# PaddlePaddle/PaddleScience

Hardware: AMD Instinct MI355X
Metric: collocation-points/sec (PDE residual+grad) (higher is better)
Workload: dtype f32

## Files before the change

include/ppsci_hip.h:

```cpp
#ifndef PPSCI_HIP_H
#define PPSCI_HIP_H

#include <stddef.h>
#include <stdint.h>

#ifdef __cplusplus
extern "C" {
#endif

#define PPSCI_MAX_IN 8
#define PPSCI_MAX_DIRS 4
#define PPSCI_MAX_OUT 8
#define PPSCI_MAX_HIDDEN 16
#define PPSCI_MAX_PROG 128
#define PPSCI_MAX_RES 8
#define PPSCI_MAX_EPARAM 8
#define PPSCI_MAX_AUX 16

enum { PPSCI_OK = 0, PPSCI_E_INVALID = -1, PPSCI_E_UNSUPPORTED = -2, PPSCI_E_LAUNCH = -3 };
enum { PPSCI_ACT_TANH = 0, PPSCI_ACT_SILU = 1, PPSCI_ACT_SIN = 2, PPSCI_ACT_SIGMOID = 3, PPSCI_ACT_COS = 4, PPSCI_ACT_GELU = 5,
       PPSCI_ACT_SWISH = 6, PPSCI_ACT_STAN = 7,
       PPSCI_ACT_RELU = 8, PPSCI_ACT_LEAKY_RELU = 9, PPSCI_ACT_ELU = 10, PPSCI_ACT_SELU = 11, PPSCI_ACT_IDENTITY = 12 };
enum { PPSCI_EMBED_NONE = 0, PPSCI_EMBED_PERIOD = 1,
       PPSCI_EMBED_STREAMS = 2 };
// ... 132 lines not shown
int64_t ppsci_taylor_step_workspace_bytes(const ppsci_mlp_desc* d, const ppsci_epilogue_desc* e, int64_t n_points);
int ppsci_taylor_step_kind(const ppsci_mlp_desc* d, const ppsci_epilogue_desc* e, int64_t n_points);
void ppsci_set_fused_step(int on);
void ppsci_set_step_tail(int mode);
void ppsci_set_tail_split(int n);
void ppsci_set_fast_program(int on);
void ppsci_set_static_program(int on);
int ppsci_epilogue_predecode(const ppsci_epilogue_desc* e, uint32_t* out256, int* n_loads);
typedef struct ppsci_step_plan ppsci_step_plan;
ppsci_step_plan* ppsci_taylor_step_plan(const ppsci_mlp_desc* d, const ppsci_epilogue_desc* e, float* params,
                                        int64_t n_points, const float* const* inputs_host, const float* const* aux_host,
                                        float* U, float* Ubar, float* residual_out, void* stash, void* workspace,
                                        int64_t workspace_bytes, float* loss_terms, float* grad);
int ppsci_taylor_step_run(ppsci_step_plan* plan, int accumulate, const ppsci_adam_args* adam, void* stream);
#define PPSCI_STEP_KEEP_FRAGMENTS 1
int ppsci_taylor_step_run_ex(ppsci_step_plan* plan, int accumulate, const ppsci_adam_args* adam, void* stream, int flags);
int ppsci_taylor_step_plan_apply(ppsci_step_plan* plan, const ppsci_adam_args* adam, void* stream);
int ppsci_taylor_step_plan_set_scales(ppsci_step_plan* plan, const ppsci_epilogue_desc* e);
int ppsci_taylor_step_run_main(ppsci_step_plan* plan, void* stream);
void ppsci_taylor_step_plan_free(ppsci_step_plan* plan);
int ppsci_taylor_step_plan_static(const ppsci_step_plan* plan, const char** name);
void ppsci_set_fused_specialised(int on);
int ppsci_taylor_step_plan_specialised(const ppsci_step_plan* plan);
int ppsci_taylor_step(const ppsci_mlp_desc* d, const ppsci_epilogue_desc* e, float* params, int64_t n_points,
                      const float* const* inputs_host, const float* const* aux_host, float* U, float* Ubar,
                      float* residual_out, void* stash, void* workspace, int64_t workspace_bytes, float* loss_terms,
                      float* grad, int accumulate, const ppsci_adam_args* adam, void* stream);

int ppsci_reduce_rows(const float* partials, int64_t rows, int64_t cols, float* out, int accumulate,
                      void* stream);

int ppsci_adam_step(int64_t n, float* params, const float* grad, float* m, float* v, float lr,
                    float beta1, float beta2, float eps, int64_t step_t, float grad_scale,
                    void* stream);

#define PPSCI_MTL_MAX_LOSSES 8
#define PPSCI_MTL_PCGRAD 0
#define PPSCI_MTL_GRAM_ONLY 1
int64_t ppsci_grad_surgery_workspace_bytes(int K, int64_t n);
int ppsci_grad_surgery(int K, int64_t n, const float* G, int64_t ld, const int32_t* order, int mode, float* gram_out,
                       float* coef_out, float* w_out, void* workspace, int64_t workspace_bytes, void* stream);
int ppsci_grad_combine(int K, int64_t n, const float* G, int64_t ld, const float* w_dev, const float* w_host, float* out,
                       float* params, const ppsci_adam_args* adam, void* stream);

#define PPSCI_OPT_SGD 0
#define PPSCI_OPT_MOMENTUM 1
// ... 314 lines not shown
```

paddlescience_amd/_lib.py:

```python
from __future__ import annotations

import ctypes as C
import os
from typing import List, Optional, Sequence

MAX_IN, MAX_DIRS, MAX_OUT, MAX_HIDDEN, MAX_PROG, MAX_RES, MAX_AUX = 8, 4, 8, 16, 128, 8, 16

ACT = {"tanh": 0, "silu": 1, "sin": 2, "sigmoid": 3, "cos": 4, "gelu": 5, "swish": 6, "stan": 7, "relu": 8, "leaky_relu": 9,
       "elu": 10, "selu": 11, "identity": 12}
PARAM_ACTS = ("swish", "stan")
SIREN_W0 = 30.0
LINEAR_PLAIN, LINEAR_WEIGHT_NORM, LINEAR_RWF, LINEAR_FOURIER, LINEAR_BROADCAST = range(5)
LINEAR_PADDED = 100
EMBED_NONE, EMBED_PERIOD, EMBED_STREAMS = 0, 1, 2

(OP_LD_IN, OP_LD_U, OP_LD_AUX, OP_CONST, OP_ADD, OP_SUB, OP_MUL, OP_DIV, OP_NEG, OP_POW, OP_SIN, OP_COS,
 OP_TANH, OP_EXP, OP_LOG, OP_SQRT, OP_ABS, OP_SINH, OP_COSH, OP_TAN, OP_MAX, OP_MIN, OP_SIGN, OP_HEAVISIDE,
 OP_DETACH, OP_ASIN, OP_ACOS, OP_ATAN, OP_ATAN2, OP_ASINH, OP_ACOSH, OP_ATANH, OP_ERF, OP_LGAMMA, OP_CEIL, OP_FLOOR,
 OP_LD_PARAM, OP_COUNT) = range(38)
MAX_EPARAM = 8
MTL_MAX_LOSSES = 8
MTL_PCGRAD, MTL_GRAM_ONLY = 0, 1
STEP_KEEP_FRAGMENTS = 1

# ... 134 lines not shown
                                        C.c_void_p, C.c_void_p]),
    "ppsci_taylor_bwd": (C.c_int, [C.POINTER(MlpDesc), C.c_void_p, C.c_int64, C.POINTER(C.c_void_p), C.c_void_p,
                                   C.c_void_p, C.c_void_p, C.c_void_p, C.c_void_p]),
    "ppsci_taylor_bwd_ws": (C.c_int, [C.POINTER(MlpDesc), C.c_void_p, C.c_int64, C.POINTER(C.c_void_p), C.c_void_p,
                                      C.c_void_p, C.c_void_p, C.c_int64, C.c_void_p, C.c_void_p]),
    "ppsci_dense_matvec": (C.c_int, [C.c_int64, C.c_int64, C.c_void_p, C.c_void_p, C.c_void_p, C.c_float, C.c_int, C.c_void_p,
                                     C.c_void_p]),
    "ppsci_csr_matvec": (C.c_int, [C.c_int64, C.c_int64, C.c_int64, C.c_void_p, C.c_void_p, C.c_void_p, C.c_void_p, C.c_void_p,
                                   C.c_float, C.c_void_p, C.c_void_p]),
    "ppsci_reduce_rows": (C.c_int, [C.c_void_p, C.c_int64, C.c_int64, C.c_void_p, C.c_int, C.c_void_p]),
    "ppsci_taylor_step_workspace_bytes": (C.c_int64, [C.POINTER(MlpDesc), C.POINTER(EpilogueDesc), C.c_int64]),
    "ppsci_taylor_step_kind": (C.c_int, [C.POINTER(MlpDesc), C.POINTER(EpilogueDesc), C.c_int64]),
    "ppsci_set_fused_step": (None, [C.c_int]),
    "ppsci_set_step_tail": (None, [C.c_int]),
    "ppsci_set_tail_split": (None, [C.c_int]),
    "ppsci_set_fast_program": (None, [C.c_int]),
    "ppsci_taylor_step_run_ex": (C.c_int, [C.c_void_p, C.c_int, C.POINTER(AdamArgs), C.c_void_p, C.c_int]),
    "ppsci_taylor_step_plan_apply": (C.c_int, [C.c_void_p, C.POINTER(AdamArgs), C.c_void_p]),
    "ppsci_set_static_program": (None, [C.c_int]),
    "ppsci_epilogue_predecode": (C.c_int, [C.POINTER(EpilogueDesc), C.POINTER(C.c_uint32), C.POINTER(C.c_int)]),
    "ppsci_taylor_step_plan_static": (C.c_int, [C.c_void_p, C.POINTER(C.c_char_p)]),
    "ppsci_set_fused_specialised": (None, [C.c_int]),
    "ppsci_taylor_step_plan_specialised": (C.c_int, [C.c_void_p]),
    "ppsci_taylor_step_plan": (C.c_void_p, [C.POINTER(MlpDesc), C.POINTER(EpilogueDesc), C.c_void_p, C.c_int64,
                                            C.POINTER(C.c_void_p), C.POINTER(C.c_void_p), C.c_void_p, C.c_void_p, C.c_void_p,
                                            C.c_void_p, C.c_void_p, C.c_int64, C.c_void_p, C.c_void_p]),
    "ppsci_taylor_step_run": (C.c_int, [C.c_void_p, C.c_int, C.POINTER(AdamArgs), C.c_void_p]),
    "ppsci_taylor_step_plan_set_scales": (C.c_int, [C.c_void_p, C.POINTER(EpilogueDesc)]),
    "ppsci_taylor_step_run_main": (C.c_int, [C.c_void_p, C.c_void_p]),
    "ppsci_taylor_step_plan_free": (None, [C.c_void_p]),
    "ppsci_taylor_step": (C.c_int, [C.POINTER(MlpDesc), C.POINTER(EpilogueDesc), C.c_void_p, C.c_int64, C.POINTER(C.c_void_p),
                                    C.POINTER(C.c_void_p), C.c_void_p, C.c_void_p, C.c_void_p, C.c_void_p, C.c_void_p,
                                    C.c_int64, C.c_void_p, C.c_void_p, C.c_int, C.POINTER(AdamArgs), C.c_void_p]),
    "ppsci_spectral_conv2d_fwd": (C.c_int, [C.POINTER(SpectralDesc), C.c_void_p, C.c_void_p, C.c_void_p, C.c_void_p,
                                            C.c_void_p]),
    "ppsci_spectral_conv2d_bwd": (C.c_int, [C.POINTER(SpectralDesc), C.c_void_p, C.c_void_p, C.c_void_p, C.c_void_p,
                                            C.c_void_p, C.c_void_p, C.c_void_p, C.c_void_p]),
    "ppsci_spectral_conv2d_bwd_real": (C.c_int, [C.POINTER(SpectralDesc), C.c_void_p, C.c_void_p, C.c_void_p, C.c_void_p,
                                                 C.c_void_p, C.c_void_p, C.c_void_p, C.c_float, C.c_int, C.c_void_p]),
    "ppsci_spectral_conv2d_fwd_scaled": (C.c_int, [C.POINTER(SpectralDesc), C.c_void_p, C.c_void_p, C.c_void_p, C.c_void_p,
                                                   C.c_float, C.c_int, C.c_void_p]),
    "ppsci_spectral_conv2d_bwd_real_scaled": (C.c_int, [C.POINTER(SpectralDesc), C.c_void_p, C.c_void_p, C.c_void_p,
                                                        C.c_void_p, C.c_void_p, C.c_void_p, C.c_void_p, C.c_float, C.c_int,
                                                        C.c_float, C.c_int, C.c_void_p]),
    "ppsci_dft2_kept_supported": (C.c_int, [C.c_int] * 4),
    "ppsci_dft2_kept_fwd": (C.c_int, [C.c_int] * 6 + [C.c_void_p] * 3),
# ... 222 lines not shown
```

paddlescience_amd/csrc/taylor_api.hip:

```cpp
#include "taylor_tile.h"
#include "taylor_step.h"
#include "epi_static.h"

#include <math.h>
#include <stdlib.h>
#include <string.h>

#include <mutex>

__global__ void __launch_bounds__(256) ppsci_presplit_kernel(const float* params, ppsci_derived q, int H, int L, int bwd,
                                                             u32x4* out) {
  const int NB = q.NB, NKP = NB / 2;
  const int per_layer = NB * NKP * 64;
  const int total = (L - 1) * per_layer;
  for (int idx = blockIdx.x * blockDim.x + threadIdx.x; idx < total; idx += gridDim.x * blockDim.x) {
    const int l = 1 + idx / per_layer, rem = idx % per_layer;
    const int lane = rem & 63, pair = rem >> 6, rb = pair / NKP, kp = pair - rb * NKP;
    const int g = lane >> 4, c = lane & 15;
    const float* W = params + q.offW[l];
    ppsci_split4 sp[2];
#pragma unroll
    for (int hlf = 0; hlf < 2; ++hlf) {
      const int kb = 2 * kp + hlf;
      f32x4 v;
// ... 290 lines not shown
  const int64_t other = ppsci_bwd_workspace_bytes(d, n_points);
  int rc;
  if (other > 0 && other <= workspace_bytes) {
    rc = taylor_bwd_impl(d, params, n_points, inputs_host, Ubar, stash, workspace, grad_partials, stream);
  } else {
    ppsci_set_error("taylor_bwd: workspace of %lld bytes, %lld needed (ppsci_bwd_workspace_bytes)", (long long)workspace_bytes,
                    (long long)need);
    rc = PPSCI_E_INVALID;
  }
  ppsci_set_bwd_layerwise(knob);
  return rc;
}

static int g_fused_step = 1, g_step_tail = -1, g_fast_vm = 1, g_static_prog = 1;
extern "C" void ppsci_set_fast_program(int on) { g_fast_vm = on ? 1 : 0; }
extern "C" void ppsci_set_static_program(int on) { g_static_prog = on ? 1 : 0; }
extern "C" int ppsci_epilogue_predecode(const ppsci_epilogue_desc* e, uint32_t* out256, int* n_loads) {
  int nl = 0;
  if (!e || !out256) return -1;
  const int n = epi_fast_encode(*e, out256, &nl);
  if (n_loads) *n_loads = nl;
  return n;
}
static int g_fused_spec = 1;
extern "C" void ppsci_set_fused_specialised(int on) { g_fused_spec = on ? 1 : 0; }
extern "C" void ppsci_set_fused_step(int on) { g_fused_step = on ? 1 : 0; }
extern "C" void ppsci_set_step_tail(int mode) { g_step_tail = (mode < 0 || mode > 3) ? -1 : mode; }
#define PPSCI_FUSED_TREE_MAX_GRID 48

static int run_step_act(StepArgs& a, void* stream, int launch, int* grid) {
  if (a.f.d.fourier_half > 0) return PPSCI_E_UNSUPPORTED;
  if (launch == 2 ? a.t.fused != 0 : g_fused_step != 0) {
    int rc = PPSCI_E_UNSUPPORTED;
    const bool st = a.e.static_id > 0;
    switch (a.f.d.activation) {
      case PPSCI_ACT_TANH: rc = st ? ppsci_fused_static_run_tanh(a, stream, launch, grid) : ppsci_fused_run_tanh(a, stream, launch, grid); break;
      case PPSCI_ACT_SILU: rc = st ? ppsci_fused_static_run_silu(a, stream, launch, grid) : ppsci_fused_run_silu(a, stream, launch, grid); break;
      case PPSCI_ACT_SIN: rc = st ? ppsci_fused_static_run_sin(a, stream, launch, grid) : ppsci_fused_run_sin(a, stream, launch, grid); break;
      default: break;
    }
    if (rc != PPSCI_E_UNSUPPORTED || launch == 2) return rc;
    a.e.static_id = 0;
  }
  a.t.fused = 0;
  switch (a.f.d.activation) {
    case PPSCI_ACT_TANH: return ppsci_step_run_tanh(a, stream, launch, grid);
    case PPSCI_ACT_SILU: return ppsci_step_run_silu(a, stream, launch, grid);
    case PPSCI_ACT_SIN: return ppsci_step_run_sin(a, stream, launch, grid);
// ... 173 lines not shown
    if (nfast >= 0) {
#ifdef PPSCI_EMU
      memcpy(ws + y.fastprog, fast, sizeof(fast));
#else
      if (hipMemcpy(ws + y.fastprog, fast, sizeof(fast), hipMemcpyHostToDevice) != hipSuccess) {
        ppsci_set_error("taylor_step: cannot upload the pre-decoded residual program");
        return fail();
      }
#endif
      a.e.fast = (const unsigned*)(ws + y.fastprog);
      a.e.nfast = nfast;
      a.e.nfast_loads = nfast_loads;
    }
  }
  a.f.params = a.b.params = params;
  for (int j = 0; j < d->d_raw; ++j) a.f.x[j] = a.b.x[j] = a.e.x[j] = inputs_host[j];
  for (int j = 0; j < e->n_aux; ++j) a.e.aux[j] = aux_host[j];
  a.f.U = U;
  a.f.stash = (f32x4*)stash;
  a.e.U = U;
  a.e.Ubar = Ubar;
  a.e.resid = residual_out;
  a.t.spec = (a.t.fused && a.t.spec_ok && g_fused_spec && !U && !Ubar && !residual_out) ? 1 : 0;
  a.e.partials = ws + y.rows_l;
  a.b.Ubar = Ubar;
  a.b.stash = (const f32x4*)stash;
  a.b.partials = ws + y.rows_s;
  a.b.wpart = (f32x4*)(ws + y.rows_w);
  StepTail& t = a.t;
  t.rows_w = ws + y.rows_w;
  t.rows_s = ws + y.rows_s;
  t.rows_l = ws + y.rows_l;
  t.tree = ws + y.tree;
  t.counters = (unsigned*)(ws + y.counters);
  t.grad = grad;
  t.loss_terms = loss_terms;
  t.p = params;
  t.per_tile = y.per_tile;
  t.psmall = y.psmall;
  t.n_res = e->n_res;
  t.rowlen = y.rowlen;
  return plan;
}

extern "C" void ppsci_taylor_step_plan_free(ppsci_step_plan* plan) { delete plan; }

extern "C" int ppsci_taylor_step_plan_static(const ppsci_step_plan* plan, const char** name) {
  const int id = plan ? plan->a.e.static_id : 0;
  if (name) *name = epi_static_name(id);
  return id;
}

extern "C" int ppsci_taylor_step_plan_specialised(const ppsci_step_plan* plan) { return plan && plan->a.t.fused && plan->a.t.spec ? 1 : 0; }

extern "C" int ppsci_taylor_step_plan_set_scales(ppsci_step_plan* plan, const ppsci_epilogue_desc* e) {
  if (!plan || !e || e->n_res != plan->a.e.e.n_res) {
    ppsci_set_error("taylor_step_plan_set_scales: invalid argument");
    return PPSCI_E_INVALID;
  }
  for (int k = 0; k < e->n_res; ++k) plan->a.e.e.res[k].scale = e->res[k].scale;
  return PPSCI_OK;
}

extern "C" int ppsci_taylor_step_run(ppsci_step_plan* plan, int accumulate, const ppsci_adam_args* adam, void* stream) {
  return ppsci_taylor_step_run_ex(plan, accumulate, adam, stream, 0);
}

extern "C" int ppsci_taylor_step_run_ex(ppsci_step_plan* plan, int accumulate, const ppsci_adam_args* adam, void* stream, int flags) {
  if (!plan) {
    ppsci_set_error("taylor_step_run: invalid argument");
    return PPSCI_E_INVALID;
  }
  StepTail& t = plan->a.t;
  t.accumulate = accumulate ? 1 : 0;
  t.do_adam = 0;
  if (adam) {
// ... 141 lines not shown
```

paddlescience_amd/csrc/taylor_fused.inc:

```
#include "taylor_tile.h"
#include "taylor_step_tail.h"
#include "epi_static.h"

#include <stdlib.h>
#include <string.h>
#include <type_traits>

#ifndef PPSCI_FUSED_STATIC
#define PPSCI_FUSED_STATIC 0
#endif
#ifndef PPSCI_FUSED_LANE_BIAS
#define PPSCI_FUSED_LANE_BIAS(L, S, ACT, STATIC) ((L) * ((S) + 1) <= (((STATIC) && (ACT) == PPSCI_ACT_TANH) ? 20 : 12))
#endif
#define PPSCI_FUSED_EPI_SCRATCH ((PPSCI_MAX_RES + PPSCI_MAX_EPARAM) * 16)
#define PPSCI_FUSED_SPEC_TAB (64 + PPSCI_MAX_RES + PPSCI_MAX_DIRS * PPSCI_FUSED_MAX_IN)
#define PPSCI_FUSED_MAX_IN 4
#define PPSCI_FUSED_XJ(x, j) ((j) == 0 ? (x)[0] : ((j) == 1 ? (x)[1] : ((j) == 2 ? (x)[2] : (x)[3])))

#ifdef PPSCI_FUSED_TIMERS
#define PPSCI_FT(k)                                             \
  {                                                             \
    const unsigned long long now_ = __builtin_amdgcn_s_memtime(); \
    tacc[k] += now_ - tlast;                                    \
    tlast = now_;                                               \
  }
#else
#define PPSCI_FT(k)
#endif

#define PPSCI_ABL(n) (((ABL) >> (n)) & 1)
template <int ABL>
__device__ __forceinline__ ppsci_split4 ppsci_fused_split(f32x4 x) {
  if (PPSCI_ABL(6)) {
    ppsci_split4 o;
    o.p[0] = (u32x2){__builtin_bit_cast(unsigned, x[0]), __builtin_bit_cast(unsigned, x[1])};
    o.p[1] = (u32x2){__builtin_bit_cast(unsigned, x[2]), __builtin_bit_cast(unsigned, x[3])};
    o.p[2] = o.p[0];
    return o;
  }
// ... 1 lines not shown
}

#ifdef PPSCI_DBG_DUMP
__device__ float* ppsci_dbg_buf = nullptr;
extern "C" int ppsci_dbg_set(float* p) { return (int)hipMemcpyToSymbol(HIP_SYMBOL(ppsci_dbg_buf), &p, sizeof(p)); }
#define PPSCI_DBG_STRIDE 16384
#endif


static inline long long ppsci_fused_floats(const ppsci_mlp_desc& d, const ppsci_derived& q, int S, int n_instr) {
  const int m = d.d_out, pad4m = ((m + 3) / 4) * 4;
  long long fl = 2LL * ((q.d0 + d.n_hidden + m) * q.HP + pad4m);
  fl += (q.NB + 1) * m * S * PPSCI_TILE;
  fl += q.NB * d.d_raw * PPSCI_TILE;
  fl += (long long)q.NB * m * S * PPSCI_TILE;
  fl += PPSCI_FUSED_EPI_SCRATCH + PPSCI_MAX_RES * PPSCI_TILE;
  fl += 2LL * n_instr * PPSCI_TILE;
  fl += EPI_FAST_WORDS + PPSCI_MAX_RES + PPSCI_MAX_RES * PPSCI_TILE;
  fl += 2LL * S * q.NB * 3 * 64 * 2;
  fl += PPSCI_MAX_DIRS * q.HP;
  return fl;
}

template <int NB, int LH, int N1, int N2, int D_RAW, int M>
static constexpr long long ppsci_fused_floats_spec() {
  constexpr int S = 1 + N1 + N2, HP = 16 * NB, pad4m = ((M + 3) / 4) * 4;
  long long fl = 2LL * ((D_RAW + LH + M) * HP + pad4m);
  fl += 2LL * NB * M * S * PPSCI_TILE;
  fl += NB * D_RAW * PPSCI_TILE;
  fl += PPSCI_FUSED_EPI_SCRATCH + PPSCI_MAX_RES * PPSCI_TILE;
  fl += PPSCI_FUSED_SPEC_TAB;
  fl += 2LL * S * NB * 3 * 64 * 2;
  fl += PPSCI_MAX_DIRS * HP;
  return fl;
}

template <int NB, int LH, int N1, int N2, int ACT, bool STATIC, int ABL = 0, int D_RAW = 0, int M = 0>
__global__ void __launch_bounds__(64 * NB, 2) taylor_fused_kernel(StepArgs args) {
  constexpr int S = 1 + N1 + N2;
  constexpr bool SPEC = D_RAW > 0;
  static_assert(!SPEC || (STATIC && M > 0 && D_RAW <= PPSCI_FUSED_MAX_IN), "shape-specialised kernels are STATIC kernels");
  constexpr int HP = 16 * NB;
  constexpr int W = NB;
  constexpr int L = LH;
  constexpr int NKP = NB / 2;
  constexpr bool LANE_BIAS = PPSCI_FUSED_LANE_BIAS(LH, S, ACT, STATIC);
  static_assert(NB == 4, "one feature block per wave, both k-pairs of a layer's fragments held in registers");
  PPSCI_DYN_SMEM(smem);
  const FwdArgs& a = args.f;
  const int tid = threadIdx.x, nthr = blockDim.x;
  const int lane = tid & 63, wave = __builtin_amdgcn_readfirstlane(tid >> 6);
  const int g = lane >> 4, c = lane & 15;
  const int H = a.d.width, m = SPEC ? M : a.d.d_out, d0 = SPEC ? D_RAW : a.q.d0, d_raw = SPEC ? D_RAW : a.d.d_raw;
  const int pad4m = ((m + 3) / 4) * 4;
  const int n_instr = SPEC ? 0 : args.e.e.n_instr;

  float* W0s = smem;
  float* Bs = W0s + d0 * HP;
  float* WLs = Bs + L * HP;
  float* BLs = WLs + m * HP;
  float* gW0 = BLs + pad4m;
  float* gB = gW0 + d0 * HP;
  float* gWL = gB + L * HP;
  float* gBL = gWL + m * HP;
  float* tin = gBL + pad4m;
  float* uls = tin + W * m * S * PPSCI_TILE;
  float* tinx = uls + (SPEC ? 0 : m * S * PPSCI_TILE);
  float* red = tinx + W * d_raw * PPSCI_TILE;
  float* ered = red + W * m * S * PPSCI_TILE;
  float* lacc = ered + PPSCI_FUSED_EPI_SCRATCH;
  float* rf = lacc + PPSCI_MAX_RES * PPSCI_TILE;
  unsigned* ftab = (unsigned*)(rf + 2 * n_instr * PPSCI_TILE);
  float* rres = (float*)(ftab + EPI_FAST_WORDS + PPSCI_MAX_RES);
  u32x2* zx = (u32x2*)(SPEC ? (float*)ftab + PPSCI_FUSED_SPEC_TAB : rres + PPSCI_MAX_RES * PPSCI_TILE);
  u32x2* hx = zx + S * NB * 3 * 64;
  float* dz0 = (float*)(hx + S * NB * 3 * 64);
  f32x4* zsave = (f32x4*)hx;
  static_assert(L * S * 64 * 16 <= S * NB * 3 * 64 * 8, "zsave must fit into hx");
  constexpr bool VM_REGS_OK = (L - 1) * NB * 64 * 16 <= S * NB * 3 * 64 * 8;
  float* prow = args.b.partials + (long long)blockIdx.x * ppsci_small_params(a.d, a.q);

  for (int idx = tid; idx < d0 * HP; idx += nthr) {
    const int k = idx / HP, f = idx - k * HP;
    W0s[idx] = (f < H) ? a.params[a.q.offW[0] + k * H + f] : 0.f;
  }
  for (int idx = tid; idx < L * HP; idx += nthr) {
    const int l = idx / HP, f = idx - l * HP;
    Bs[idx] = (f < H) ? a.params[a.q.offB[l] + f] : 0.f;
  }
  for (int idx = tid; idx < m * HP; idx += nthr) {
    const int cc = idx / HP, f = idx - cc * HP;
    WLs[idx] = (f < H) ? a.params[a.q.offW[L] + f * m + cc] : 0.f;
  }
  for (int idx = tid; idx < pad4m; idx += nthr) BLs[idx] = idx < m ? a.params[a.q.offB[L] + idx] : 0.f;
  bool raw_only = true;
  if constexpr (!SPEC)
    for (int j = 0; j < d_raw; ++j) raw_only = raw_only && a.d.embed[j] == PPSCI_EMBED_NONE;
  if (raw_only)
    for (int idx = tid; idx < N1 * HP; idx += nthr) {
// ... 116 lines not shown
#pragma unroll
            for (int i = 0; i < N2; ++i) d2v[i] = ddv * a.d.dirs[i][j] * a.d.dirs[i][j];
          }
          const f32x4 w4 = *(const f32x4*)&W0s[k * HP + 16 * wave + 4 * g];
          h[0] += w4 * val;
#pragma unroll
          for (int i = 0; i < N1; ++i) h[1 + i] += w4 * d1v[i];
#pragma unroll
          for (int i = 0; i < N2; ++i) h[1 + N1 + i] += w4 * d2v[i];
        }
      }
      h[0] += *(const f32x4*)&Bs[16 * wave + 4 * g];
    }

    PPSCI_FT(1)
    auto fwd_layer = [&](auto lc) {
      constexpr int l = decltype(lc)::value;
      int lanel = lane;
      PPSCI_OPAQUE(lanel);
      const int g = lanel >> 4;
      const int xcl = ppsci_xchunk(lanel >> 4, lanel & 15);
      if constexpr (l > 0) {
        u32x2* xb = STATIC ? (((L - 1 - l) & 1) ? zx : hx) : ((l & 1) ? zx : hx);
        if constexpr (STATIC && l == 1 && (L % 2) == 0) ppsci_block_sync_lds();
        const u32x4* gf = (const u32x4*)a.xfrag + (long long)(l - 1) * PPSCI_GFRAG_PER_LAYER(NB) + lanel;
        u32x4 Ak[NKP][3];
#pragma unroll
        for (int kp = 0; kp < NKP; ++kp)
#pragma unroll
          for (int q = 0; q < 3; ++q) Ak[kp][q] = gf[((wave * NKP + kp) * 3 + q) * 64];
#pragma unroll
        for (int s = 0; s < S; ++s) {
          const ppsci_split4 sp = ppsci_fused_split<ABL>(h[s]);
#pragma unroll
          for (int q = 0; q < 3; ++q)
            if (!PPSCI_ABL(9) || (sp.p[q][0] == 0x12345u && sp.p[q][1] == 0x54321u)) xb[ppsci_xpair(NB, s, wave, q, xcl)] = sp.p[q];
        }
        __builtin_amdgcn_sched_barrier(0);
        ppsci_block_sync_lds();
        PPSCI_FT(2)
        h[0] = *(const f32x4*)&Bs[l * HP + 16 * wave + 4 * g];
#pragma unroll
        for (int s = 1; s < S; ++s) h[s] = (f32x4){0.f, 0.f, 0.f, 0.f};
        {
          u32x4 bq[2][S];
          const auto load_b = [&](int grp, u32x4 (&dst)[S]) {
            const int kp = grp / 3, pb = 2 - grp % 3;
#pragma unroll
            for (int s = 0; s < S; ++s) dst[s] = *(const u32x4*)&xb[ppsci_xpair(NB, s, 2 * kp, pb, xcl)];
          };
          load_b(0, bq[0]);
#pragma unroll
          for (int grp = 0; grp < 3 * NKP; ++grp) {
            const int kp = grp / 3, pb = 2 - grp % 3;
            if (grp + 1 < 3 * NKP) load_b(grp + 1, bq[(grp + 1) & 1]);
            __builtin_amdgcn_sched_barrier(0);
#pragma unroll
            for (int pa = 2 - pb; pa >= 0; --pa)
#pragma unroll
              for (int s = 0; s < S; ++s) {
                const u32x4 bb = bq[grp & 1][s];
                if (PPSCI_ABL(5)) h[s][0] += __builtin_bit_cast(float, bb[0] ^ Ak[kp][pa][0]) * 1e-30f;
// ... 365 lines not shown
            const int kp = grp / 3, pb = 2 - grp % 3;
            if (grp + 1 < 3 * NKP) load_b(grp + 1, bq[(grp + 1) & 1]);
            __builtin_amdgcn_sched_barrier(0);
#pragma unroll
            for (int pa = 2 - pb; pa >= 0; --pa)
#pragma unroll
              for (int s = 0; s < S; ++s) {
                const u32x4 bb = bq[grp & 1][s];
                if (PPSCI_ABL(4)) hb[s][0] += __builtin_bit_cast(float, bb[0] ^ Ab[kp][pa][0]) * 1e-30f;
                else
                hb[s] = ppsci_xdl32a(Ab[kp][pa], (u32x2){bb[0], bb[1]}, (u32x2){bb[2], bb[3]}, hb[s]);
              }
            __builtin_amdgcn_sched_barrier(0);
          }
        }
#ifdef PPSCI_DBG_DUMP
        if (ppsci_dbg_buf != nullptr && l == L - 1) {
#pragma unroll
          for (int s = 0; s < S; ++s) *(f32x4*)&ppsci_dbg_buf[(long long)blockIdx.x * PPSCI_DBG_STRIDE + 8192 + (s * 256 + tid) * 4] = hb[s];
        }
#endif
        PPSCI_FT(8)
        constexpr bool HPAIR = STATIC && l == L - 1;
        if (!PPSCI_ABL(3) && !HPAIR) {
          f32x4 E1, E2, E3;
          f32x4 hcs[S];
          if (PPSCI_ABL(7)) {
            hcs[0] = zst[l - 1][0];
            E1 = (f32x4){0.5f, 0.5f, 0.5f, 0.5f}, E2 = (f32x4){0.1f, 0.1f, 0.1f, 0.1f};
          } else
            ppsci_act_from_stash4<ACT>(zst[l - 1][0], hcs[0], E1, E2, E3);
#pragma unroll
          for (int i = 0; i < N1; ++i) {
            hcs[1 + i] = E1 * zst[l - 1][1 + i];
            if (i < N2) hcs[1 + N1 + i] = E2 * zst[l - 1][1 + i] * zst[l - 1][1 + i] + E1 * zst[l - 1][1 + N1 + i];
          }
#pragma unroll
          for (int s = 0; s < S; ++s) {
            const ppsci_split4 sp = ppsci_fused_split<ABL>(hcs[s]);
#pragma unroll
            for (int q = 0; q < 3; ++q)
              if (!PPSCI_ABL(9) || (sp.p[q][0] == 0x12345u && sp.p[q][1] == 0x54321u)) hx[((s * NB + wave) * 3 + q) * 64 + xcl] = sp.p[q];
            __builtin_amdgcn_sched_barrier(0);
          }
        }
        __builtin_amdgcn_sched_barrier(0);
        if (!PPSCI_ABL(3)) ppsci_block_sync_lds();
        PPSCI_FT(9)
#pragma unroll 1
        for (int sp = 0; sp + 1 < (PPSCI_ABL(3) ? 0 : S); sp += 2) {
          int zs_ = ppsci_xpair(NB, sp, wave, 0, xtl);
          int hs_ = HPAIR ? ppsci_xpair(NB, sp, 0, 0, xtl) : xtl + sp * NB * 3 * 64;
          PPSCI_OPAQUE(zs_);
          PPSCI_OPAQUE(hs_);
          u32x2 zN0[3], zN1[3];
#pragma unroll
          for (int q = 0; q < 3; ++q) {
            zN0[q] = ppsci_lds_read_tr16(&zx[zs_ + q * 128]);
            zN1[q] = ppsci_lds_read_tr16(&zx[zs_ + (NKP * 3 + q) * 128]);
          }
          constexpr int IG = 2;
          u32x2 hN0[2][IG][3], hN1[2][IG][3];
          const auto load_h = [&](int ig, int buf) {
#pragma unroll
            for (int e = 0; e < IG; ++e)
#pragma unroll
              for (int q = 0; q < 3; ++q) {
                if constexpr (HPAIR) {
                  hN0[buf][e][q] = ppsci_lds_read_tr16(&hx[hs_ + (((ig + e) >> 1) * 3 + q) * 128 + ((ig + e) & 1)]);
                  hN1[buf][e][q] = ppsci_lds_read_tr16(&hx[hs_ + ((NKP + ((ig + e) >> 1)) * 3 + q) * 128 + ((ig + e) & 1)]);
                } else {
                  hN0[buf][e][q] = ppsci_lds_read_tr16(&hx[hs_ + ((ig + e) * 3 + q) * 64]);
                  hN1[buf][e][q] = ppsci_lds_read_tr16(&hx[hs_ + ((NB + ig + e) * 3 + q) * 64]);
                }
              }
          };
          load_h(0, 0);
#pragma unroll
          for (int ig = 0; ig < NB; ig += IG) {
            const int buf = (ig / IG) & 1;
            if (ig + IG < NB) load_h(ig + IG, buf ^ 1);
            __builtin_amdgcn_sched_barrier(0);
#pragma unroll
            for (int q = 0; q < PPSCI_XDL_NPROD; ++q)
#pragma unroll
              for (int e = 0; e < IG; ++e)
                wacc[l - 1][ig + e] = ppsci_xdl32(hN0[buf][e][ppsci_xdl_pa[q]], hN1[buf][e][ppsci_xdl_pa[q]], zN0[ppsci_xdl_pb[q]],
                                                  zN1[ppsci_xdl_pb[q]], wacc[l - 1][ig + e]);
            __builtin_amdgcn_sched_barrier(0);
          }
        }
        if constexpr (S & 1) {
          u32x2 zN0[3];
#pragma unroll
          for (int q = 0; q < 3; ++q) zN0[q] = ppsci_lds_read_tr16(&zx[ppsci_xpair(NB, S - 1, wave, q, xtl)]);
          u32x2 hN0[NB][3];
#pragma unroll
          for (int e = 0; e < NB; ++e)
#pragma unroll
            for (int q = 0; q < 3; ++q)
              hN0[e][q] = ppsci_lds_read_tr16(HPAIR ? &hx[ppsci_xpair(NB, S - 1, e, q, xtl)] : &hx[(((S - 1) * NB + e) * 3 + q) * 64 + xtl]);
#pragma unroll
          for (int q = 0; q < PPSCI_XDL_NPROD; ++q)
#pragma unroll
            for (int e = 0; e < NB; ++e)
              wacc[l - 1][e] = ppsci_xdl16(hN0[e][ppsci_xdl_pa[q]], zN0[ppsci_xdl_pb[q]], wacc[l - 1][e]);
          __builtin_amdgcn_sched_barrier(0);
        }
        PPSCI_FT(10)
      } else {
        PPSCI_FT(7)
        const long long p = (long long)tile * PPSCI_TILE + c;
        const long long pp = p < a.N ? p : 0;
        const float vm = p < a.N ? 1.f : 0.f;
        int k = 0;
        if constexpr (STATIC) {
#pragma unroll
          for (int j = 0; j < PPSCI_FUSED_MAX_IN; ++j) {
            if (j < d_raw && !PPSCI_ABL(0)) {
              f32x4 t = hb[0] * tx[j * PPSCI_TILE + c];
#pragma unroll
              for (int i = 0; i < N1; ++i) t += hb[1 + i] * (SPEC ? dirs_s[i * D_RAW + j] : a.d.dirs[i][j]);
              f32x4 v4;
#pragma unroll
// ... 105 lines not shown
  }
  for (int idx = tid; idx < H * m; idx += nthr) {
    const int f = idx / m, cc = idx - f * m;
    ppsci_store_agent(&prow[(d0 + L) * H + idx], gWL[cc * HP + f]);
  }
  for (int idx = tid; idx < m; idx += nthr) ppsci_store_agent(&prow[(d0 + L + m) * H + idx], gBL[idx]);
  {
    float lsum[PPSCI_MAX_RES], padj[PPSCI_MAX_EPARAM];
#pragma unroll
    for (int k = 0; k < PPSCI_MAX_RES; ++k) lsum[k] = (wave == 0 && lane < PPSCI_TILE) ? lacc[k * PPSCI_TILE + lane] : 0.f;
#pragma unroll
    for (int k = 0; k < PPSCI_MAX_EPARAM; ++k) padj[k] = 0.f;
    epi_finale<EPI_RF_FUSED>(args.e, ered, lsum, padj);
  }
  if (args.t.external != 1) ppsci_step_tail(args.t, args.b.d, args.b.q, smem);
}

#if PPSCI_FUSED_STATIC && defined(PPSCI_FUSED_SPEC_D_RAW) && !defined(PPSCI_ABL_BUILD)
#define PPSCI_FUSED_HAS_SPEC 1
#define PPSCI_FUSED_SPEC_KERNEL (taylor_fused_kernel<NB, LH, N1, N2, PPSCI_ACT_ID, true, 0, PPSCI_FUSED_SPEC_D_RAW, PPSCI_FUSED_SPEC_M>)
#else
#define PPSCI_FUSED_HAS_SPEC 0
#endif

template <int NB, int LH, int N1, int N2>
static int launch_fused(StepArgs& a, void* stream, int launch, int* grid_out) {
  constexpr int S = 1 + N1 + N2;
#if PPSCI_FUSED_HAS_SPEC
  constexpr int lds_spec = (int)(ppsci_fused_floats_spec<NB, LH, N1, N2, PPSCI_FUSED_SPEC_D_RAW, PPSCI_FUSED_SPEC_M>() * 4);
#endif
  if (launch == 2) {
#if PPSCI_FUSED_HAS_SPEC
    if (a.t.spec) {
      PPSCI_LAUNCH(PPSCI_FUSED_SPEC_KERNEL, StepArgs, a.t.grid, 64 * NB, lds_spec, stream, a);
      int e = PPSCI_LAST_LAUNCH_ERROR();
      if (e != 0) {
        ppsci_set_error("taylor_fused: launch failed (hip error %d)", e);
        return PPSCI_E_LAUNCH;
      }
      return PPSCI_OK;
    }
#endif
#ifdef PPSCI_ABL_BUILD
    {
      const char* ev = getenv("PPSCI_ABL");
      const int mask = ev ? atoi(ev) : 0;
#define PPSCI_ABL_CASE(M_)                                                                                                          \
  if (mask == (M_)) {                                                                                                               \
    PPSCI_SET_MAX_LDS((taylor_fused_kernel<NB, LH, N1, N2, PPSCI_ACT_ID, PPSCI_FUSED_STATIC != 0, (M_)>), a.t.lds);                    \
    PPSCI_LAUNCH((taylor_fused_kernel<NB, LH, N1, N2, PPSCI_ACT_ID, PPSCI_FUSED_STATIC != 0, (M_)>), StepArgs, a.t.grid, 64 * NB, a.t.lds, \
                 stream, a);                                                                                                        \
    return PPSCI_LAST_LAUNCH_ERROR() != 0 ? PPSCI_E_LAUNCH : PPSCI_OK;                                                              \
  }
      PPSCI_ABL_CASE(1) PPSCI_ABL_CASE(2) PPSCI_ABL_CASE(4) PPSCI_ABL_CASE(8) PPSCI_ABL_CASE(16) PPSCI_ABL_CASE(32) PPSCI_ABL_CASE(64)
      PPSCI_ABL_CASE(128) PPSCI_ABL_CASE(256) PPSCI_ABL_CASE(512)
#undef PPSCI_ABL_CASE
    }
#endif
    PPSCI_LAUNCH((taylor_fused_kernel<NB, LH, N1, N2, PPSCI_ACT_ID, PPSCI_FUSED_STATIC != 0>), StepArgs, a.t.grid, 64 * NB, a.t.lds, stream, a);
    int e = PPSCI_LAST_LAUNCH_ERROR();
    if (e != 0) {
      ppsci_set_error("taylor_fused: launch failed (hip error %d)", e);
      return PPSCI_E_LAUNCH;
    }
    return PPSCI_OK;
  }
  const long long fl = ppsci_fused_floats(a.f.d, a.f.q, S, a.e.e.n_instr);
  if (fl * 4 > PPSCI_LDS_LIMIT_BYTES / 2) {
    ppsci_set_error("taylor_fused: LDS need %lld B exceeds half a CU", fl * 4);
    return PPSCI_E_UNSUPPORTED;
  }
  const int lds = (int)(fl * 4);
  if (PPSCI_SET_MAX_LDS((taylor_fused_kernel<NB, LH, N1, N2, PPSCI_ACT_ID, PPSCI_FUSED_STATIC != 0>), lds) != 0) {
    ppsci_set_error("taylor_fused: cannot raise dynamic LDS to %d B", lds);
    return PPSCI_E_LAUNCH;
  }
  a.t.spec = a.t.spec_ok = 0;
#if PPSCI_FUSED_HAS_SPEC
  if (a.f.d.d_raw == PPSCI_FUSED_SPEC_D_RAW && a.f.q.d0 == PPSCI_FUSED_SPEC_D_RAW && a.f.d.d_out == PPSCI_FUSED_SPEC_M && lds_spec <= lds &&
      PPSCI_SET_MAX_LDS(PPSCI_FUSED_SPEC_KERNEL, lds_spec) == 0)
    a.t.spec_ok = 1;
#endif
  int per_cu = 1;
  if (PPSCI_OCCUPANCY((taylor_fused_kernel<NB, LH, N1, N2, PPSCI_ACT_ID, PPSCI_FUSED_STATIC != 0>), 64 * NB, lds, &per_cu) != 0 || per_cu < 1) per_cu = 1;
  const int ntl = a.f.ntiles;
  int grid = ntl < PPSCI_NUM_CU * per_cu ? ntl : PPSCI_NUM_CU * per_cu;
  if (ppsci_get_max_grid() > 0 && grid > ppsci_get_max_grid()) grid = ppsci_get_max_grid();
  if (grid < 1) grid = 1;
  a.f.iters = a.b.iters = a.e.iters = (ntl + grid - 1) / grid;
  a.f.tile0 = a.b.tile0 = 0;
  a.f.resident = a.b.resident = 1;
  a.b.accum = 1;
  a.b.xdl_split = 1;
  a.t.grid = grid;
  a.t.lds = lds;
  a.t.fused = 1;
  if (grid_out) *grid_out = grid;
  if (!launch) return PPSCI_OK;
  PPSCI_LAUNCH((taylor_fused_kernel<NB, LH, N1, N2, PPSCI_ACT_ID, PPSCI_FUSED_STATIC != 0>), StepArgs, grid, 64 * NB, lds, stream, a);
  int e = PPSCI_LAST_LAUNCH_ERROR();
  if (e != 0) {
    ppsci_set_error("taylor_fused: launch failed (hip error %d)", e);
    return PPSCI_E_LAUNCH;
  }
  return PPSCI_OK;
}

// ... 31 lines not shown
```

paddlescience_amd/csrc/taylor_fused_static_tanh.hip:

```cpp
#ifndef PPSCI_SPLIT_CONST_VGPR
#define PPSCI_SPLIT_CONST_VGPR 1
#endif
#define PPSCI_ACT_ID PPSCI_ACT_TANH
#define PPSCI_FUSED_STATIC 1
#define PPSCI_FUSED_SPEC_D_RAW 2
#define PPSCI_FUSED_SPEC_M 1
#define PPSCI_FUSED_RUN_NAME ppsci_fused_static_run_tanh
#include "taylor_fused.inc"
```

paddlescience_amd/csrc/taylor_step.h:

```cpp
#pragma once
#include "epilogue_vm.h"

#ifdef PPSCI_EMU
#define PPSCI_STEP_FAN 3
#else
#define PPSCI_STEP_FAN 16
#endif

struct StepTail {
  float* rows_w;
  float* rows_s;
  float* rows_l;
  float* tree;
  unsigned* counters;
  float* grad;
  float* loss_terms;
  float* p;
  float* m;
  float* v;
  int grid, per_tile, psmall, n_res, rowlen;
  int lds;
  int accumulate, do_adam;
  float lr_t, beta1, beta2, eps_t, grad_scale;
  int fused;
  int spec_ok, spec;
  int one_tail;
  int external;
};

struct StepArgs {
  FwdArgs f;
  BwdArgs b;
  EpiArgs e;
  StepTail t;
};

int ppsci_step_run_tanh(StepArgs& a, void* stream, int launch, int* grid_out);
int ppsci_step_run_silu(StepArgs& a, void* stream, int launch, int* grid_out);
int ppsci_step_run_sin(StepArgs& a, void* stream, int launch, int* grid_out);
int ppsci_fused_run_tanh(StepArgs& a, void* stream, int launch, int* grid_out);
int ppsci_fused_run_silu(StepArgs& a, void* stream, int launch, int* grid_out);
int ppsci_fused_run_sin(StepArgs& a, void* stream, int launch, int* grid_out);
int ppsci_fused_static_run_tanh(StepArgs& a, void* stream, int launch, int* grid_out);
int ppsci_fused_static_run_silu(StepArgs& a, void* stream, int launch, int* grid_out);
int ppsci_fused_static_run_sin(StepArgs& a, void* stream, int launch, int* grid_out);
```

paddlescience_amd/hotpath.py:

```python
from __future__ import annotations

import ctypes as C
from dataclasses import dataclass, field
from typing import Dict, List, Optional, Sequence, Tuple

import torch

from . import _lib as L


def _stream_ptr(t: torch.Tensor):
    if t.is_cuda:
        return C.c_void_p(torch._C._cuda_getCurrentRawStream(t.device.index))
    return None


def _p(t: Optional[torch.Tensor]):
    return None if t is None else C.c_void_p(t.data_ptr())


def _chk_f32(*ts):
    for t in ts:
        if t is not None and (t.dtype != torch.float32 or not t.is_contiguous()):
            raise ValueError("hot-path buffers must be contiguous float32 tensors")
# ... 176 lines not shown
        keep = (not capturing and self._frag_token is not None
                and self._frag_token == (_PARAM_WRITES[0], self._params._version))
        L.check(self._run(self.handle, 1 if accumulate else 0, aa, _stream_ptr(self._dev), L.STEP_KEEP_FRAGMENTS if keep else 0))
        if adam is not None:
            note_param_write()
        self._frag_token = None if capturing else (_PARAM_WRITES[0], self._params._version)

    def apply_adam(self, adam: dict) -> None:
        aa = _adam_args(adam)
        L.check(L.lib().ppsci_taylor_step_plan_apply(self.handle, C.byref(aa), _stream_ptr(self._dev)))
        note_param_write()
        capturing = self._params.is_cuda and torch.cuda.is_current_stream_capturing()
        self._frag_token = None if capturing else (_PARAM_WRITES[0], self._params._version)

    @property
    def static_program(self) -> str:
        nm = C.c_char_p()
        return (nm.value or b"").decode() if L.lib().ppsci_taylor_step_plan_static(self.handle, C.byref(nm)) > 0 else ""

    @property
    def specialised(self) -> bool:
        return L.lib().ppsci_taylor_step_plan_specialised(self.handle) == 1

    def run_main(self) -> None:
        L.check(L.lib().ppsci_taylor_step_run_main(self.handle, _stream_ptr(self._dev)))

    def __del__(self):
        h, self.handle = getattr(self, "handle", None), None
        if h:
            self._free(h)


_PARAM_WRITES = [0]


def note_param_write() -> None:
    _PARAM_WRITES[0] += 1


def dense_matvec(M: torch.Tensor, x: torch.Tensor, y: torch.Tensor, alpha: float = 1.0, transpose: bool = False,
                 rowscale: Optional[torch.Tensor] = None) -> None:
    _require_device(y)
    _chk_f32(M, x, y, rowscale)
    rows, cols = M.shape
    assert x.numel() >= (rows if transpose else cols) and y.numel() >= (cols if transpose else rows)
    L.check(L.lib().ppsci_dense_matvec(rows, cols, _p(M), _p(x), _p(rowscale), float(alpha), 1 if transpose else 0, _p(y),
# ... 243 lines not shown
```

Measured before the change: 474.1 million.

## Keep forward activation planes in LDS for backward pass in specialised fused kernel

Adds a KEEP variant of the shape-specialised fused Taylor kernel. It stores the split hidden-activation planes of layer L-2 (and optionally layer 1) in an extra LDS buffer during the forward pass, so the backward pass reads them directly instead of recomputing and re-splitting them. The epilogue scratch is aliased into zx to offset the extra LDS. The variant is enabled only when it fits the LDS budget and keeps the same occupancy. It can also drop one block sync for even-depth networks.

```diff
diff --git a/include/ppsci_hip.h b/include/ppsci_hip.h
--- a/include/ppsci_hip.h
+++ b/include/ppsci_hip.h
@@ -178,6 +178,8 @@
 int ppsci_taylor_step_plan_static(const ppsci_step_plan* plan, const char** name);
 void ppsci_set_fused_specialised(int on);
 int ppsci_taylor_step_plan_specialised(const ppsci_step_plan* plan);
+void ppsci_set_fused_keep_planes(int on);
+int ppsci_taylor_step_plan_keep_planes(const ppsci_step_plan* plan);
 int ppsci_taylor_step(const ppsci_mlp_desc* d, const ppsci_epilogue_desc* e, float* params, int64_t n_points,
                       const float* const* inputs_host, const float* const* aux_host, float* U, float* Ubar,
                       float* residual_out, void* stash, void* workspace, int64_t workspace_bytes, float* loss_terms,
diff --git a/paddlescience_amd/_lib.py b/paddlescience_amd/_lib.py
--- a/paddlescience_amd/_lib.py
+++ b/paddlescience_amd/_lib.py
@@ -180,6 +180,8 @@
     "ppsci_taylor_step_plan_static": (C.c_int, [C.c_void_p, C.POINTER(C.c_char_p)]),
     "ppsci_set_fused_specialised": (None, [C.c_int]),
     "ppsci_taylor_step_plan_specialised": (C.c_int, [C.c_void_p]),
+    "ppsci_set_fused_keep_planes": (None, [C.c_int]),
+    "ppsci_taylor_step_plan_keep_planes": (C.c_int, [C.c_void_p]),
     "ppsci_taylor_step_plan": (C.c_void_p, [C.POINTER(MlpDesc), C.POINTER(EpilogueDesc), C.c_void_p, C.c_int64,
                                             C.POINTER(C.c_void_p), C.POINTER(C.c_void_p), C.c_void_p, C.c_void_p, C.c_void_p,
                                             C.c_void_p, C.c_void_p, C.c_int64, C.c_void_p, C.c_void_p]),
diff --git a/paddlescience_amd/csrc/taylor_api.hip b/paddlescience_amd/csrc/taylor_api.hip
--- a/paddlescience_amd/csrc/taylor_api.hip
+++ b/paddlescience_amd/csrc/taylor_api.hip
@@ -336,8 +336,9 @@
   if (n_loads) *n_loads = nl;
   return n;
 }
-static int g_fused_spec = 1;
+static int g_fused_spec = 1, g_fused_keep = 1;
 extern "C" void ppsci_set_fused_specialised(int on) { g_fused_spec = on ? 1 : 0; }
+extern "C" void ppsci_set_fused_keep_planes(int on) { g_fused_keep = on ? 1 : 0; }
 extern "C" void ppsci_set_fused_step(int on) { g_fused_step = on ? 1 : 0; }
 extern "C" void ppsci_set_step_tail(int mode) { g_step_tail = (mode < 0 || mode > 3) ? -1 : mode; }
 #define PPSCI_FUSED_TREE_MAX_GRID 48
@@ -557,6 +558,7 @@
   a.e.Ubar = Ubar;
   a.e.resid = residual_out;
   a.t.spec = (a.t.fused && a.t.spec_ok && g_fused_spec && !U && !Ubar && !residual_out) ? 1 : 0;
+  a.t.keep = (a.t.spec && a.t.keep_ok && g_fused_keep) ? 1 : 0;
   a.e.partials = ws + y.rows_l;
   a.b.Ubar = Ubar;
   a.b.stash = (const f32x4*)stash;
@@ -587,6 +589,9 @@
 }
 
 extern "C" int ppsci_taylor_step_plan_specialised(const ppsci_step_plan* plan) { return plan && plan->a.t.fused && plan->a.t.spec ? 1 : 0; }
+extern "C" int ppsci_taylor_step_plan_keep_planes(const ppsci_step_plan* plan) {
+  return plan && plan->a.t.fused && plan->a.t.spec && plan->a.t.keep ? 1 : 0;
+}
 
 extern "C" int ppsci_taylor_step_plan_set_scales(ppsci_step_plan* plan, const ppsci_epilogue_desc* e) {
   if (!plan || !e || e->n_res != plan->a.e.e.n_res) {
diff --git a/paddlescience_amd/csrc/taylor_fused.inc b/paddlescience_amd/csrc/taylor_fused.inc
--- a/paddlescience_amd/csrc/taylor_fused.inc
+++ b/paddlescience_amd/csrc/taylor_fused.inc
@@ -15,6 +15,9 @@
 #define PPSCI_FUSED_EPI_SCRATCH ((PPSCI_MAX_RES + PPSCI_MAX_EPARAM) * 16)
 #define PPSCI_FUSED_SPEC_TAB (64 + PPSCI_MAX_RES + PPSCI_MAX_DIRS * PPSCI_FUSED_MAX_IN)
 #define PPSCI_FUSED_MAX_IN 4
+#ifndef PPSCI_FUSED_KEEP_H0
+#define PPSCI_FUSED_KEEP_H0 1
+#endif
 #define PPSCI_FUSED_XJ(x, j) ((j) == 0 ? (x)[0] : ((j) == 1 ? (x)[1] : ((j) == 2 ? (x)[2] : (x)[3])))
 
 #ifdef PPSCI_FUSED_TIMERS
@@ -62,24 +65,30 @@
   return fl;
 }
 
-template <int NB, int LH, int N1, int N2, int D_RAW, int M>
+template <int NB, int LH, int N1, int N2, int D_RAW, int M, bool KEEP = false>
 static constexpr long long ppsci_fused_floats_spec() {
   constexpr int S = 1 + N1 + N2, HP = 16 * NB, pad4m = ((M + 3) / 4) * 4;
   long long fl = 2LL * ((D_RAW + LH + M) * HP + pad4m);
   fl += 2LL * NB * M * S * PPSCI_TILE;
   fl += NB * D_RAW * PPSCI_TILE;
-  fl += PPSCI_FUSED_EPI_SCRATCH + PPSCI_MAX_RES * PPSCI_TILE;
+  fl += (KEEP ? 0 : PPSCI_FUSED_EPI_SCRATCH) + PPSCI_MAX_RES * PPSCI_TILE;
   fl += PPSCI_FUSED_SPEC_TAB;
-  fl += 2LL * S * NB * 3 * 64 * 2;
-  fl += PPSCI_MAX_DIRS * HP;
+  fl += (KEEP ? 3LL : 2LL) * S * NB * 3 * 64 * 2;
+  fl += (KEEP ? N1 : PPSCI_MAX_DIRS) * HP;
   return fl;
 }
-
-template <int NB, int LH, int N1, int N2, int ACT, bool STATIC, int ABL = 0, int D_RAW = 0, int M = 0>
+template <int NB, int LH, int N1, int N2, int D_RAW, int M>
+static constexpr bool ppsci_fused_keep_fits() {
+  return LH >= 3 && 4 * ppsci_fused_floats_spec<NB, LH, N1, N2, D_RAW, M, true>() <= PPSCI_LDS_LIMIT_BYTES / 2;
+}
+
+template <int NB, int LH, int N1, int N2, int ACT, bool STATIC, int ABL = 0, int D_RAW = 0, int M = 0, bool KEEP = false>
 __global__ void __launch_bounds__(64 * NB, 2) taylor_fused_kernel(StepArgs args) {
   constexpr int S = 1 + N1 + N2;
   constexpr bool SPEC = D_RAW > 0;
   static_assert(!SPEC || (STATIC && M > 0 && D_RAW <= PPSCI_FUSED_MAX_IN), "shape-specialised kernels are STATIC kernels");
+  static_assert(!KEEP || (SPEC && LH >= 3 && ABL == 0), "planes are kept by shape-specialised kernels with a layer L-2 >= 1");
+  constexpr bool KEEP_H0 = KEEP && PPSCI_FUSED_KEEP_H0 != 0 && (LH % 2) == 0 && LH >= 4;
   constexpr int HP = 16 * NB;
   constexpr int W = NB;
   constexpr int L = LH;
@@ -108,13 +117,16 @@
   float* tinx = uls + (SPEC ? 0 : m * S * PPSCI_TILE);
   float* red = tinx + W * d_raw * PPSCI_TILE;
   float* ered = red + W * m * S * PPSCI_TILE;
-  float* lacc = ered + PPSCI_FUSED_EPI_SCRATCH;
+  float* lacc = ered + (KEEP ? 0 : PPSCI_FUSED_EPI_SCRATCH);
   float* rf = lacc + PPSCI_MAX_RES * PPSCI_TILE;
   unsigned* ftab = (unsigned*)(rf + 2 * n_instr * PPSCI_TILE);
   float* rres = (float*)(ftab + EPI_FAST_WORDS + PPSCI_MAX_RES);
   u32x2* zx = (u32x2*)(SPEC ? (float*)ftab + PPSCI_FUSED_SPEC_TAB : rres + PPSCI_MAX_RES * PPSCI_TILE);
   u32x2* hx = zx + S * NB * 3 * 64;
-  float* dz0 = (float*)(hx + S * NB * 3 * 64);
+  u32x2* kx = hx + S * NB * 3 * 64;
+  float* dz0 = (float*)(hx + (KEEP ? 2 : 1) * S * NB * 3 * 64);
+  if constexpr (KEEP) ered = (float*)zx;
+  static_assert(!KEEP || PPSCI_FUSED_EPI_SCRATCH * 4 <= S * NB * 3 * 64 * 8, "ered must fit into zx");
   f32x4* zsave = (f32x4*)hx;
   static_assert(L * S * 64 * 16 <= S * NB * 3 * 64 * 8, "zsave must fit into hx");
   constexpr bool VM_REGS_OK = (L - 1) * NB * 64 * 16 <= S * NB * 3 * 64 * 8;
@@ -277,7 +289,9 @@
       const int xcl = ppsci_xchunk(lanel >> 4, lanel & 15);
       if constexpr (l > 0) {
         u32x2* xb = STATIC ? (((L - 1 - l) & 1) ? zx : hx) : ((l & 1) ? zx : hx);
-        if constexpr (STATIC && l == 1 && (L % 2) == 0) ppsci_block_sync_lds();
+        if constexpr (STATIC && l == 1 && (L % 2) == 0 && !KEEP_H0) ppsci_block_sync_lds();
+        constexpr bool KFWD = KEEP && l == L - 2, KLATE = KFWD && l == 1;
+        ppsci_split4 spk[KLATE ? S : 1];
         const u32x4* gf = (const u32x4*)a.xfrag + (long long)(l - 1) * PPSCI_GFRAG_PER_LAYER(NB) + lanel;
         u32x4 Ak[NKP][3];
 #pragma unroll
@@ -290,9 +304,20 @@
 #pragma unroll
           for (int q = 0; q < 3; ++q)
             if (!PPSCI_ABL(9) || (sp.p[q][0] == 0x12345u && sp.p[q][1] == 0x54321u)) xb[ppsci_xpair(NB, s, wave, q, xcl)] = sp.p[q];
+          if constexpr (KLATE) spk[s] = sp;
+          else if constexpr (KFWD) {
+#pragma unroll
+            for (int q = 0; q < 3; ++q) kx[((s * NB + wave) * 3 + q) * 64 + xcl] = sp.p[q];
+          }
         }
         __builtin_amdgcn_sched_barrier(0);
         ppsci_block_sync_lds();
+        if constexpr (KLATE) {
+#pragma unroll
+          for (int s = 0; s < S; ++s)
+#pragma unroll
+            for (int q = 0; q < 3; ++q) kx[((s * NB + wave) * 3 + q) * 64 + xcl] = spk[s].p[q];
+        }
         PPSCI_FT(2)
         h[0] = *(const f32x4*)&Bs[l * HP + 16 * wave + 4 * g];
 #pragma unroll
@@ -704,7 +729,9 @@
 #endif
         PPSCI_FT(8)
         constexpr bool HPAIR = STATIC && l == L - 1;
-        if (!PPSCI_ABL(3) && !HPAIR) {
+        constexpr bool HKEPT = KEEP && l == L - 2;
+        u32x2* const ha = (HKEPT || (KEEP_H0 && l == 1)) ? kx : hx;
+        if (!PPSCI_ABL(3) && !HPAIR && !HKEPT) {
           f32x4 E1, E2, E3;
           f32x4 hcs[S];
           if (PPSCI_ABL(7)) {
@@ -722,7 +749,7 @@
             const ppsci_split4 sp = ppsci_fused_split<ABL>(hcs[s]);
 #pragma unroll
             for (int q = 0; q < 3; ++q)
-              if (!PPSCI_ABL(9) || (sp.p[q][0] == 0x12345u && sp.p[q][1] == 0x54321u)) hx[((s * NB + wave) * 3 + q) * 64 + xcl] = sp.p[q];
+              if (!PPSCI_ABL(9) || (sp.p[q][0] == 0x12345u && sp.p[q][1] == 0x54321u)) ha[((s * NB + wave) * 3 + q) * 64 + xcl] = sp.p[q];
             __builtin_amdgcn_sched_barrier(0);
           }
         }
@@ -752,8 +779,8 @@
                   hN0[buf][e][q] = ppsci_lds_read_tr16(&hx[hs_ + (((ig + e) >> 1) * 3 + q) * 128 + ((ig + e) & 1)]);
                   hN1[buf][e][q] = ppsci_lds_read_tr16(&hx[hs_ + ((NKP + ((ig + e) >> 1)) * 3 + q) * 128 + ((ig + e) & 1)]);
                 } else {
-                  hN0[buf][e][q] = ppsci_lds_read_tr16(&hx[hs_ + ((ig + e) * 3 + q) * 64]);
-                  hN1[buf][e][q] = ppsci_lds_read_tr16(&hx[hs_ + ((NB + ig + e) * 3 + q) * 64]);
+                  hN0[buf][e][q] = ppsci_lds_read_tr16(&ha[hs_ + ((ig + e) * 3 + q) * 64]);
+                  hN1[buf][e][q] = ppsci_lds_read_tr16(&ha[hs_ + ((NB + ig + e) * 3 + q) * 64]);
                 }
               }
           };
@@ -781,7 +808,7 @@
           for (int e = 0; e < NB; ++e)
 #pragma unroll
             for (int q = 0; q < 3; ++q)
-              hN0[e][q] = ppsci_lds_read_tr16(HPAIR ? &hx[ppsci_xpair(NB, S - 1, e, q, xtl)] : &hx[(((S - 1) * NB + e) * 3 + q) * 64 + xtl]);
+              hN0[e][q] = ppsci_lds_read_tr16(HPAIR ? &hx[ppsci_xpair(NB, S - 1, e, q, xtl)] : &ha[(((S - 1) * NB + e) * 3 + q) * 64 + xtl]);
 #pragma unroll
           for (int q = 0; q < PPSCI_XDL_NPROD; ++q)
 #pragma unroll
@@ -933,6 +960,12 @@
 #else
 #define PPSCI_FUSED_HAS_SPEC 0
 #endif
+#if PPSCI_FUSED_HAS_SPEC && defined(PPSCI_FUSED_KEEP_PLANES) && PPSCI_FUSED_KEEP_PLANES && !defined(PPSCI_FUSED_TIMERS)
+#define PPSCI_FUSED_HAS_KEEP 1
+#define PPSCI_FUSED_KEEP_KERNEL (taylor_fused_kernel<NB, LH, N1, N2, PPSCI_ACT_ID, true, 0, PPSCI_FUSED_SPEC_D_RAW, PPSCI_FUSED_SPEC_M, true>)
+#else
+#define PPSCI_FUSED_HAS_KEEP 0
+#endif
 
 template <int NB, int LH, int N1, int N2>
 static int launch_fused(StepArgs& a, void* stream, int launch, int* grid_out) {
@@ -943,6 +976,12 @@
   if (launch == 2) {
 #if PPSCI_FUSED_HAS_SPEC
     if (a.t.spec) {
+#if PPSCI_FUSED_HAS_KEEP
+      if constexpr (ppsci_fused_keep_fits<NB, LH, N1, N2, PPSCI_FUSED_SPEC_D_RAW, PPSCI_FUSED_SPEC_M>()) {
+        if (a.t.keep) PPSCI_LAUNCH(PPSCI_FUSED_KEEP_KERNEL, StepArgs, a.t.grid, 64 * NB, a.t.lds_keep, stream, a);
+        else PPSCI_LAUNCH(PPSCI_FUSED_SPEC_KERNEL, StepArgs, a.t.grid, 64 * NB, lds_spec, stream, a);
+      } else
+#endif
       PPSCI_LAUNCH(PPSCI_FUSED_SPEC_KERNEL, StepArgs, a.t.grid, 64 * NB, lds_spec, stream, a);
       int e = PPSCI_LAST_LAUNCH_ERROR();
       if (e != 0) {
@@ -986,7 +1025,7 @@
     ppsci_set_error("taylor_fused: cannot raise dynamic LDS to %d B", lds);
     return PPSCI_E_LAUNCH;
   }
-  a.t.spec = a.t.spec_ok = 0;
+  a.t.spec = a.t.spec_ok = a.t.keep = a.t.keep_ok = a.t.lds_keep = 0;
 #if PPSCI_FUSED_HAS_SPEC
   if (a.f.d.d_raw == PPSCI_FUSED_SPEC_D_RAW && a.f.q.d0 == PPSCI_FUSED_SPEC_D_RAW && a.f.d.d_out == PPSCI_FUSED_SPEC_M && lds_spec <= lds &&
       PPSCI_SET_MAX_LDS(PPSCI_FUSED_SPEC_KERNEL, lds_spec) == 0)
@@ -994,6 +1033,17 @@
 #endif
   int per_cu = 1;
   if (PPSCI_OCCUPANCY((taylor_fused_kernel<NB, LH, N1, N2, PPSCI_ACT_ID, PPSCI_FUSED_STATIC != 0>), 64 * NB, lds, &per_cu) != 0 || per_cu < 1) per_cu = 1;
+#if PPSCI_FUSED_HAS_KEEP
+  if constexpr (ppsci_fused_keep_fits<NB, LH, N1, N2, PPSCI_FUSED_SPEC_D_RAW, PPSCI_FUSED_SPEC_M>()) {
+    constexpr int lds_keep = (int)(ppsci_fused_floats_spec<NB, LH, N1, N2, PPSCI_FUSED_SPEC_D_RAW, PPSCI_FUSED_SPEC_M, true>() * 4);
+    int pc = 0;
+    if (a.t.spec_ok && PPSCI_SET_MAX_LDS(PPSCI_FUSED_KEEP_KERNEL, lds_keep) == 0 &&
+        PPSCI_OCCUPANCY(PPSCI_FUSED_KEEP_KERNEL, 64 * NB, lds_keep, &pc) == 0 && pc == per_cu) {
+      a.t.keep_ok = 1;
+      a.t.lds_keep = lds_keep;
+    }
+  }
+#endif
   const int ntl = a.f.ntiles;
   int grid = ntl < PPSCI_NUM_CU * per_cu ? ntl : PPSCI_NUM_CU * per_cu;
   if (ppsci_get_max_grid() > 0 && grid > ppsci_get_max_grid()) grid = ppsci_get_max_grid();
diff --git a/paddlescience_amd/csrc/taylor_fused_static_tanh.hip b/paddlescience_amd/csrc/taylor_fused_static_tanh.hip
--- a/paddlescience_amd/csrc/taylor_fused_static_tanh.hip
+++ b/paddlescience_amd/csrc/taylor_fused_static_tanh.hip
@@ -5,5 +5,8 @@
 #define PPSCI_FUSED_STATIC 1
 #define PPSCI_FUSED_SPEC_D_RAW 2
 #define PPSCI_FUSED_SPEC_M 1
+#ifndef PPSCI_FUSED_KEEP_PLANES
+#define PPSCI_FUSED_KEEP_PLANES 1
+#endif
 #define PPSCI_FUSED_RUN_NAME ppsci_fused_static_run_tanh
 #include "taylor_fused.inc"
diff --git a/paddlescience_amd/csrc/taylor_step.h b/paddlescience_amd/csrc/taylor_step.h
--- a/paddlescience_amd/csrc/taylor_step.h
+++ b/paddlescience_amd/csrc/taylor_step.h
@@ -24,6 +24,8 @@
   float lr_t, beta1, beta2, eps_t, grad_scale;
   int fused;
   int spec_ok, spec;
+  int keep_ok, keep;
+  int lds_keep;
   int one_tail;
   int external;
 };
diff --git a/paddlescience_amd/hotpath.py b/paddlescience_amd/hotpath.py
--- a/paddlescience_amd/hotpath.py
+++ b/paddlescience_amd/hotpath.py
@@ -222,6 +222,10 @@
     def specialised(self) -> bool:
         return L.lib().ppsci_taylor_step_plan_specialised(self.handle) == 1
 
+    @property
+    def keep_planes(self) -> bool:
+        return L.lib().ppsci_taylor_step_plan_keep_planes(self.handle) == 1
+
     def run_main(self) -> None:
         L.check(L.lib().ppsci_taylor_step_run_main(self.handle, _stream_ptr(self._dev)))
 
```

New measurement: 483.5 million (median of 6 runs). 2.0% higher.
